# s-elkazdadi/ddp-pinocchio

Measured on AMD Instinct MI355X. Metric: DDP iterations/sec (fwd+bwd sweep), Talos nq=38 T=200, higher is better.
Workload: dtype f64

## Files before the change

ddp_pinocchio_amd/csrc/fwd.hip:

```cpp
#include <math.h>
#include <stdio.h>
#include <stdlib.h>

#include <type_traits>
#include <vector>

#include "com_cost.h"
#include "control_grav_cost.h"
#include "frame_aim_cost.h"
#include "frame_cost.h"
#include "frame_vel_cost.h"
#include "internal.h"
#include "momentum_cost.h"
#include "obstacle_cost.h"
#include "rbd.h"
#include "relative_frame_cost.h"
#include "self_collision_cost.h"
#include "state_limits.h"

namespace {

struct FwdParams {
  Dims d;
  const DevModel* model;
// ... 281 lines not shown
      const double* wu = p.wu + ((int64_t)b * T + t) * nv;
      for (int j = h; j < nv; j += NH) { const double du = u[j] - ur[j]; if (wu[j] != 0.0) su += wu[j] * du * du; }
    }
  }
  double v = 0.5 * s + 0.5 * su;
#pragma unroll
  for (int k = NH / 2; k >= 1; k /= 2) v += __shfl_xor(v, k, NH);
  return v;
}

template <bool FF, class M>
__device__ __forceinline__ double frame_lanes_sum(const FwdParams& p, const M& cm, int b, int64_t t, const double* x, int h, bool live) {
  constexpr int NH = 16;
  double s = 0;
  if (live && h < p.fc.nf) s = frame_term(p.fc, cm, FF, h, (int64_t)b * (p.d.T + 1) + t, x);
  double v = 0.5 * s;
#pragma unroll
  for (int k = NH / 2; k >= 1; k /= 2) v += __shfl_xor(v, k, NH);
  return v;
}

template <bool FF, class M>
__device__ __forceinline__ double frame_orient_lanes_sum(const FwdParams& p, const M& cm, int b, int64_t t, const double* x, int h, bool live) {
  constexpr int NH = 16;
  static_assert(2 * DDP_HIP_MAX_COST_FRAMES <= NH, "a lane per frame and kind of term");
  double s = 0;
  if (live) {
    if (h < DDP_HIP_MAX_COST_FRAMES) { if (h < p.fc.nf && p.fc.target) s = frame_term(p.fc, cm, FF, h, (int64_t)b * (p.d.T + 1) + t, x); }
    else if (h - DDP_HIP_MAX_COST_FRAMES < p.fc.nf) s = frame_orient_term(p.fc, cm, FF, h - DDP_HIP_MAX_COST_FRAMES, (int64_t)b * (p.d.T + 1) + t, x);
  }
  double v = 0.5 * s;
#pragma unroll
  for (int k = NH / 2; k >= 1; k /= 2) v += __shfl_xor(v, k, NH);
  return v;
}

template <bool FF>
__device__ __forceinline__ double limit_lanes_sum(const FwdParams& p, int b, int64_t t, const double* x, int h, bool live) {
  const int nv = (int)p.d.nv, n = 2 * nv, nq = (int)p.d.nx - nv, r0 = FF ? 6 : 0;
  constexpr int NH = 16;
  const int64_t bt1 = (int64_t)b * (p.d.T + 1) + t;
  const double* w = p.sl.weight + bt1 * n;
  const double* lo = p.sl.lo + bt1 * n;
  const double* hi = p.sl.hi + bt1 * n;
  double s = 0;
  if (live)
    for (int i = r0 + h; i < n; i += NH) {
      const double wi = w[i];
      if (wi == 0.0) continue;
      const double e = limit_excess(x[limit_coord(i, nv, nq)], lo[i], hi[i]);
      if (e != 0.0) s += wi * e * e;
    }
  double v = 0.5 * s;
#pragma unroll
  for (int k = NH / 2; k >= 1; k /= 2) v += __shfl_xor(v, k, NH);
  return v;
}

template <int NJ>
struct FwdLat2Lds {
  static constexpr int NC = 4, NH = 16, n = 2 * NJ + 1, nu = NJ;
  double state[rbd::ABA_LDS_SLOTS * (NJ + NJ / 8) * NC];
  double K[nu * n];
  double k[nu], uo[nu], xo[n];
  double dx[NC * n], x[NC * n], u[NC * nu], qdd[NC * nu];
  rbd::CoopModel<NJ> model;
};

template <int NJ>
struct FwdLat2LdsBox : FwdLat2Lds<NJ> {
  double lo[NJ], hi[NJ];
};

template <int NJ>
struct FwdPipeLds {
  static constexpr int NC = 2, NH = 16, n = 2 * NJ + 1, nu = NJ;
  double rec[2][rbd::ABA_PIPE_QSLOTS * NJ * NC];
  double z[rbd::ABA_PIPE_ZSLOTS * NJ * NC];
  double state[rbd::ABA_PIPE_XSLOTS * NJ * NC];
  double K[nu * n];
  double k[nu], uo[nu], xo[n];
  double dx[NC * n], x[2 * NC * n], u[NC * nu], qdd[NC * nu];
  rbd::CoopModel<NJ> model;
};
template <int NJ>
struct FwdPipeLdsBox : FwdPipeLds<NJ> {
  double lo[NJ], hi[NJ];
};

static bool fwd_use_pipe(const ddp_hip_ctx* ctx, int64_t batch, int n_alpha) {
  return !ctx->sw.fwd_no_pipe && batch * ((n_alpha + 1) / 2) <= ctx->cu_count;
}

#ifdef FWD_STAMPS
__device__ unsigned long long g_fwd_stamps[24];
#endif

template <int NJ, bool OPEN = false, bool FF = false, int COST = 0, bool BOX = false, bool PIPE = false>
__global__ __launch_bounds__(128) void forward_kernel_lat2(FwdParams p) {
  static_assert(!(OPEN && BOX), "the open-loop rollout applies U as given");
  constexpr bool TRACK = (COST & 1) != 0, FRAME = (COST & 2) != 0, LIMIT = (COST & 4) != 0, ORIENT = (COST & 8) != 0;
  static_assert(!ORIENT || FRAME, "the orientation terms are of the cost frames: bit 3 implies bit 1");
  using L = typename std::conditional<PIPE, typename std::conditional<BOX, FwdPipeLdsBox<NJ>, FwdPipeLds<NJ>>::type,
                                      typename std::conditional<BOX, FwdLat2LdsBox<NJ>, FwdLat2Lds<NJ>>::type>::type;
  constexpr int NC = L::NC, NH = L::NH;
  constexpr int n = 2 * NJ, nq = FF ? NJ + 1 : NJ, nx = nq + NJ, nu = NJ, XS = L::n;
  constexpr int K2 = nu * n / 2, KR = (K2 + 63) / 64;
  static_assert((nu * n) % 2 == 0, "K_t is moved in 16-byte words");
  extern __shared__ __attribute__((aligned(16))) double lds[];
  L& S = *reinterpret_cast<L*>(lds);
  const int na = OPEN ? 1 : p.n_alpha;
  const int groups = PIPE ? (na + NC - 1) / NC : 2;
  const int b = OPEN ? blockIdx.x : blockIdx.x / groups, half = OPEN ? 0 : blockIdx.x % groups;
  if (!OPEN && p.state[b] != 0) return;
  if (half * NC >= na) return;
  const int wave = threadIdx.x / 64, tid = threadIdx.x % 64, al0 = tid / NH, h = tid % NH;
  const int al = al0 < NC ? al0 : NC - 1;
  const int a = half * NC + al;
  const int cand = p.round * na + a;
  const bool mine = al0 < NC && a < na;
  const bool live = mine && cand <= 33;
  if (!OPEN && mine && cand > 33 && h == 0 && wave == 0) p.fw_dcost[(int64_t)b * na + a] = INFINITY;
  const double step = ldexp(1.0, -cand);
  const int64_t T = p.d.T;
  const double* xo = p.x_old + (int64_t)b * (T + 1) * nx;
  const double* uo = p.u_old + (int64_t)b * T * nu;
  double* xw = OPEN ? const_cast<double*>(p.x_old) + (int64_t)b * (T + 1) * nx : p.fw_x + ((int64_t)b * na + (a < na ? a : 0)) * (T + 1) * nx;
  double* uw = OPEN ? nullptr : p.fw_u + ((int64_t)b * na + (a < na ? a : 0)) * T * nu;
  const double* cold = p.costs_old + (int64_t)b * (T + 1);
  const double* kg = p.fb_val + (int64_t)b * T * nu;
  const double* Kg = p.fb_jac + (int64_t)b * T * nu * n;
  double* dx = S.dx + al * XS;
  double* x = S.x + al * XS;
  double* u = S.u + al * nu;
  double* qdd = S.qdd + al * nu;
  if (wave == 0) {
    const DevModel& m = *p.model;
    rbd::CoopModel<NJ>& cm = S.model;
    for (int i = tid; i < NJ; i += 64) {
      for (int k2 = 0; k2 < 21; ++k2) cm.I6[i][k2] = m.I6[i][k2];
      for (int k2 = 0; k2 < 9; ++k2) cm.Rp[i][k2] = m.Rp[i][k2];
      for (int k2 = 0; k2 < 3; ++k2) { cm.axis[i][k2] = m.axis[i][k2]; cm.pp[i][k2] = m.pp[i][k2]; }
      cm.parent[i] = m.parent[i]; cm.jtype[i] = m.jtype[i];
      cm.lvl_joint[i] = m.lvl_joint[i]; cm.child_list[i] = m.child_list[i];
      cm.lvl_start[i] = m.lvl_start[i]; cm.child_start[i] = m.child_start[i];
    }
    if (tid == 0) {
      cm.lvl_start[NJ] = m.lvl_start[NJ]; cm.child_start[NJ] = m.child_start[NJ];
      cm.n_levels = m.n_levels; cm.nv = m.nv; cm.nj = m.nj;
      cm.gravity[0] = m.gravity[0]; cm.gravity[1] = m.gravity[1]; cm.gravity[2] = m.gravity[2];
      cm.dt = m.dt; cm.c = m.c;
    }
    for (int e = tid; e < 16 * NH; e += 64) {
      const int L = e / NH, hh = e % NH;
      unsigned long long r = 255;
      if (L < m.n_levels && m.lvl_start[L] + hh < m.lvl_start[L + 1]) {
        const int j = m.lvl_joint[m.lvl_start[L] + hh];
        int ch[rbd::ROLE_MAX_CHILDREN] = {0, 0, 0};
        const int nch = m.child_start[j + 1] - m.child_start[j];
        for (int c = 0; c < nch && c < rbd::ROLE_MAX_CHILDREN; ++c) ch[c] = m.child_list[m.child_start[j] + c];
        r = rbd::coop_role(j, m.parent[j], m.jtype[j] == DDP_HIP_JOINT_REVOLUTE, nch, ch);
      }
      cm.role[e] = r;
    }
  }
  typedef double d2 __attribute__((ext_vector_type(2)));
  d2 Kreg[KR];
  double kreg = 0.0, uoreg = 0.0, xoreg0 = 0.0, xoreg1 = 0.0, coldreg = 0.0;
  [[maybe_unused]] double loreg = 0.0, hireg = 0.0;
  auto request = [&](int64_t t) {
    const int iu = tid < nu ? tid : nu - 1;
    uoreg = uo[t * nu + iu];
    if constexpr (!OPEN) {
      const d2* Kt = reinterpret_cast<const d2*>(Kg + t * nu * n);
#pragma unroll
      for (int j = 0; j < KR; ++j) { const int e = j * 64 + tid; Kreg[j] = Kt[e < K2 ? e : K2 - 1]; }
      kreg = kg[t * nu + iu];
      if constexpr (BOX) { loreg = p.ctrl_lo[((int64_t)b * T + t) * nu + iu]; hireg = p.ctrl_hi[((int64_t)b * T + t) * nu + iu]; }
      xoreg0 = xo[t * nx + (tid < nx ? tid : nx - 1)];
      xoreg1 = xo[t * nx + (64 + tid < nx ? 64 + tid : nx - 1)];
      coldreg = cold[t];
    }
  };
  auto park = [&]() {
    if (tid < nu) S.uo[tid] = uoreg;
    if constexpr (!OPEN) {
      d2* Ks = reinterpret_cast<d2*>(S.K);
#pragma unroll
      for (int j = 0; j < KR; ++j) { const int e = j * 64 + tid; if (e < K2) Ks[e] = Kreg[j]; }
      if (tid < nu) S.k[tid] = kreg;
      if constexpr (BOX) { if (tid < nu) { S.lo[tid] = loreg; S.hi[tid] = hireg; } }
      if (tid < nx) S.xo[tid] = xoreg0;
      if (64 + tid < nx) S.xo[64 + tid] = xoreg1;
    }
  };
  static_assert(nx <= 128, "x_old is parked by two words per lane");
  double cold_t = 0.0, dsum = 0.0;
  const double mc = p.model->c, mdt = p.model->dt;
  if (wave == 0) {
    request(0);
    const double* x0 = OPEN ? xw : p.x_new + (int64_t)b * (T + 1) * nx;
    if (live)
      for (int i = h; i < nx; i += NH) { const double v = x0[i]; x[i] = v; if (!OPEN) xw[i] = v; }
    park();
    cold_t = coldreg;
  }
  rbd::wg_sync_lds();
  const bool lead = wave == 0;
  rbd::FwdStamp* fs = nullptr;
#ifdef FWD_STAMPS
  rbd::FwdStamp fsv{};
  if (lead || PIPE) fs = &fsv;
  fsv.last = wall_clock64();
#endif
  for (int64_t t = PIPE ? -1 : 0; t < T; ++t) {
    if constexpr (PIPE) x = S.x + ((int)(t & 1) * NC + al) * XS;
    if (lead && (!PIPE || t >= 0)) {
    if constexpr (OPEN) {
      if (live)
        for (int i = h; i < nu; i += NH) u[i] = S.uo[i];
    } else {
    if constexpr (FF) {
      if (live) {
        if (h == 0) lie::se3_difference(S.xo, x, dx);
        for (int i = 6 + h; i < NJ; i += NH) dx[i] = x[i + 1] - S.xo[i + 1];
        for (int i = h; i < NJ; i += NH) dx[NJ + i] = x[nq + i] - S.xo[nq + i];
      }
    } else {
    if (live)
      for (int i = h; i < n; i += NH) dx[i] = x[i] - S.xo[i];
    }
    rbd::coop_sync<true>();
    {
      constexpr int NR = (nu + NH - 1) / NH;
      double acc[NR];
#pragma unroll
      for (int r = 0; r < NR; ++r) acc[r] = 0.0;
      const double* Kr[NR];
#pragma unroll
      for (int r = 0; r < NR; ++r) { const int i = h + NH * r; Kr[r] = S.K + (i < nu ? i : nu - 1); }
#pragma unroll
      for (int l = 0; l < n; ++l) {
        const double d = dx[l];
#pragma unroll
        for (int r = 0; r < NR; ++r) acc[r] += Kr[r][l * nu] * d;
      }
#pragma unroll
      for (int r = 0; r < NR; ++r) {
        const int i = h + NH * r;
        if (i < nu && live) {
          double ui = S.uo[i] + step * S.k[i];
          ui += acc[r];
          if constexpr (BOX) { const double lo = S.lo[i], hi = S.hi[i]; ui = ui < lo ? lo : (ui > hi ? hi : ui); }
          u[i] = ui;
          uw[t * nu + i] = ui;
        }
      }
    }
    rbd::coop_sync<true>();
    FSTAMP(fs, 0);
    double c_track = 0.0;
    if constexpr (TRACK) c_track = track_lanes_sum<FF>(p, b, t, x, u, h, live);
    if constexpr (FRAME && !ORIENT) c_track += frame_lanes_sum<FF>(p, S.model, b, t, x, h, live);
    if constexpr (ORIENT) c_track += frame_orient_lanes_sum<FF>(p, S.model, b, t, x, h, live);
    if constexpr (LIMIT) c_track += limit_lanes_sum<FF>(p, b, t, x, h, live);
    if (h == 0 && live && p.cost_inline) {
      double un = 0;
      for (int i = 0; i < nu; ++i) un += u[i] * u[i];
      double c_new = 0.5 * mc * un;
      if constexpr (TRACK || FRAME || LIMIT) c_new += c_track;
      dsum += c_new - cold_t;
    }
    }
    rbd::coop_sync<true>();
    FSTAMP(fs, 1);
    if (t + 1 < T) request(t + 1);
    FSTAMP(fs, 2);
    }
    if constexpr (PIPE) {
      double* xn = S.x + ((int)((t + 1) & 1) * NC + al) * XS;
      if (lead) {
        if (t >= 0) {
          rbd::aba_pipe_x<NJ, NC, NH, rbd::CoopModel<NJ>, FF>(S.model, S.rec[t & 1], x + nq, u, qdd, S.state, al, h, live, fs);
          if (live)
            for (int i = h; i < NJ; i += NH) {
              const double vn = x[nq + i] + qdd[i] * mdt;
              xn[nq + i] = vn;
              xw[(t + 1) * nx + nq + i] = vn;
            }
          FSTAMP(fs, 7);
          if (t + 1 < T) { park(); cold_t = coldreg; }
          FSTAMP(fs, 8);
        }
      } else {
        if (t >= 0) {
          if constexpr (FF) {
            if (live && h == 0) {
              double dq[6], q7[7];
#pragma unroll
              for (int k = 0; k < 6; ++k) dq[k] = mdt * x[nq + k];
              lie::se3_integrate(x, dq, q7);
#pragma unroll
              for (int k = 0; k < 7; ++k) xn[k] = q7[k];
            }
            if (live)
              for (int i = 6 + h; i < NJ; i += NH) { const double vo = mdt * x[nq + i]; xn[i + 1] = x[i + 1] + vo; }
          } else {
            if (live)
              for (int i = h; i < NJ; i += NH) { const double vo = mdt * x[NJ + i]; xn[i] = x[i] + vo; }
          }
          rbd::coop_sync<true>();
          FSTAMP(fs, 0);
        }
        if (t + 1 < T) rbd::aba_pipe_q<NJ, NC, NH, rbd::CoopModel<NJ>, FF>(S.model, xn, S.rec[(t + 1) & 1], S.z, al, h, live, fs);
      }
      rbd::wg_sync_lds();
      FSTAMP(fs, lead ? 3 : 5);
      if (lead && t >= 0 && live)
        for (int i = h; i < nq; i += NH) xw[(t + 1) * nx + i] = xn[i];
      continue;
    }
    rbd::aba_tree_coop2w<NJ, NC, NH, rbd::CoopModel<NJ>, FF>(S.model, x, x + nq, u, qdd, S.state, al, h, live, wave, fs);
    if (!lead) continue;
    if constexpr (FF) {
      double q7[7];
      if (live && h == 0) {
        double dq[6];
#pragma unroll
        for (int k = 0; k < 6; ++k) dq[k] = mdt * x[nq + k];
        lie::se3_integrate(x, dq, q7);
      }
      rbd::coop_sync<true>();
      if (live) {
        for (int i = 6 + h; i < NJ; i += NH) { const double vo = mdt * x[nq + i]; const double qn = x[i + 1] + vo; x[i + 1] = qn; xw[(t + 1) * nx + i + 1] = qn; }
        for (int i = h; i < NJ; i += NH) { const double vn = x[nq + i] + qdd[i] * mdt; x[nq + i] = vn; xw[(t + 1) * nx + nq + i] = vn; }
        if (h == 0) {
#pragma unroll
          for (int k = 0; k < 7; ++k) { x[k] = q7[k]; xw[(t + 1) * nx + k] = q7[k]; }
        }
      }
    } else {
    if (live)
      for (int i = h; i < NJ; i += NH) {
        const double vo = mdt * x[NJ + i];
        const double qn = x[i] + vo;
        const double vn = x[NJ + i] + qdd[i] * mdt;
        x[i] = qn; x[NJ + i] = vn;
        xw[(t + 1) * nx + i] = qn; xw[(t + 1) * nx + NJ + i] = vn;
      }
    }
    FSTAMP(fs, 7);
    if (t + 1 < T) { park(); cold_t = coldreg; }
    rbd::coop_sync<true>();
    FSTAMP(fs, 8);
  }
#ifdef FWD_STAMPS
  if (tid == 0 && blockIdx.x == 0)
    for (int i = 0; i < 12; ++i) g_fwd_stamps[12 * wave + i] = PIPE || lead ? fsv.acc[i] : 0;
#endif
  if constexpr (PIPE) x = S.x + ((int)(T & 1) * NC + al) * XS;
  double c_term = 0.0;
  if constexpr (TRACK) { if (lead) c_term = track_lanes_sum<FF>(p, b, T, x, u, h, live); }
  if constexpr (FRAME && !ORIENT) { if (lead) c_term += frame_lanes_sum<FF>(p, S.model, b, T, x, h, live); }
  if constexpr (ORIENT) { if (lead) c_term += frame_orient_lanes_sum<FF>(p, S.model, b, T, x, h, live); }
  if constexpr (LIMIT) { if (lead) c_term += limit_lanes_sum<FF>(p, b, T, x, h, live); }
  if (!OPEN && h == 0 && live && lead && p.cost_inline) {
    dsum += c_term - cold[T];
    p.fw_dcost[(int64_t)b * na + a] = dsum;
  }
}

template <int NJ, int FRAME = 0, bool LIMIT = false>
__global__ void cand_cost_kernel(FwdParams p) {
  const int64_t gid = (int64_t)blockIdx.x * blockDim.x + threadIdx.x;
  const int64_t T = p.d.T;
  const int na = p.n_alpha;
  if (gid >= p.d.batch * na * (T + 1)) return;
  const int64_t t = gid % (T + 1);
  const int a = (int)((gid / (T + 1)) % na);
  const int b = (int)(gid / ((T + 1) * na));
  if (p.state[b] != 0 || p.round * na + a > 33) return;
  const DevModel& m = *p.model;
  const int nx = m.nq + m.nv, nu = m.nv;
  const double* xs = p.fw_x + (((int64_t)b * na + a) * (T + 1) + t) * nx;
  double x[2 * NJ + 1], u[NJ];
  for (int i = 0; i < nx; ++i) x[i] = xs[i];
  double* out = p.fw_cost + ((int64_t)b * na + a) * (T + 1) + t;
  if (t == T) { *out = terminal_cost<FRAME, LIMIT>(p, m, b, x); return; }
  const double* us = p.fw_u + (((int64_t)b * na + a) * T + t) * nu;
  for (int i = 0; i < nu; ++i) u[i] = us[i];
  *out = stage_cost<NJ, FRAME, LIMIT>(p, m, b, t, x, u, p.mu[b]);
}
__global__ void cand_sum_kernel(FwdParams p) {
  const int gid = blockIdx.x * blockDim.x + threadIdx.x;
  const int na = p.n_alpha;
  if (gid >= p.d.batch * na) return;
  const int b = gid / na, a = gid % na;
  if (p.state[b] != 0 || p.round * na + a > 33) return;
  const int64_t T = p.d.T;
  const double* cold = p.costs_old + (int64_t)b * (T + 1);
  const double* cnew = p.fw_cost + ((int64_t)b * na + a) * (T + 1);
  double dsum = 0.0;
  for (int64_t t = 0; t < T; ++t) dsum += cnew[t] - cold[t];
  dsum += cnew[T] - cold[T];
  p.fw_dcost[(int64_t)b * na + a] = dsum;
}

struct CostPair {
  int64_t traj, b, bt1;
  int t;
  bool skip, live;
};
__device__ __forceinline__ CostPair cost_pair_decode(int64_t e, int64_t count, int32_t T1, int32_t na, const int32_t* state, int32_t round) {
  CostPair p{0, 0, 0, 0, true, e < count};
  if (p.live) {
    p.traj = e / T1;
    p.t = (int)(e % T1);
    p.b = p.traj / na;
    if (state && (state[p.b] != 0 || round * na + (int)(p.traj % na) > 33)) p.live = false;
    p.bt1 = p.b * T1 + p.t;
  }
  p.skip = !p.live;
  return p;
}
__device__ __forceinline__ void cost_pair_store(double* out, int64_t e, double sum, bool any, int32_t add) {
  if (add) { if (any) out[e] += sum; }
  else out[e] = sum;
}
template <int L, bool MIN, class Form>
__device__ __forceinline__ void pair_lanes_fold(double* s_term, int32_t* s_formed, int n, const double* xs, int64_t traj_stride, int64_t count,
                                                int32_t T1, int32_t nx, int32_t na, const int32_t* state, int32_t round, double* out, int32_t add,
                                                Form form) {
  const int tid = threadIdx.x, g = tid / L, k = tid % L;
  const int64_t e = (int64_t)blockIdx.x * (64 / L) + g;
  const CostPair pr = cost_pair_decode(e, count, T1, na, state, round);
  double term = MIN ? INFINITY : 0.0;
  bool formed = false;
  if (pr.live && k < n) formed = form(k, pr.bt1, xs + pr.traj * traj_stride + (int64_t)pr.t * nx, &term);
  s_term[tid] = term;
  if (!MIN) s_formed[tid] = formed ? 1 : 0;
  __syncthreads();
  if (k != 0 || pr.skip) return;
  double acc = MIN ? INFINITY : 0.0;
  bool any = false;
  for (int i = 0; i < n; ++i) {
    if (MIN) acc = rbd::obstacle_min(acc, s_term[tid + i]);
    else if (s_formed[tid + i]) { acc += s_term[tid + i]; any = true; }
  }
  cost_pair_store(out, e, acc, any, add);
// ... 345 lines not shown
#define LAT2_ROW(FF, COST) {{&forward_kernel_lat2<38, false, FF, COST, false, false>, &forward_kernel_lat2<38, false, FF, COST, false, true>}, \
                            {&forward_kernel_lat2<38, false, FF, COST, true, false>, &forward_kernel_lat2<38, false, FF, COST, true, true>}}
  static const Lat2Fn table[2][12][2][2] = {{LAT2_ROW(false, 0), LAT2_ROW(false, 1), LAT2_ROW(false, 2), LAT2_ROW(false, 3),
                                             LAT2_ROW(false, 4), LAT2_ROW(false, 5), LAT2_ROW(false, 6), LAT2_ROW(false, 7),
                                             LAT2_ROW(false, 10), LAT2_ROW(false, 11), LAT2_ROW(false, 14), LAT2_ROW(false, 15)},
                                            {LAT2_ROW(true, 0), LAT2_ROW(true, 1), LAT2_ROW(true, 2), LAT2_ROW(true, 3),
                                             LAT2_ROW(true, 4), LAT2_ROW(true, 5), LAT2_ROW(true, 6), LAT2_ROW(true, 7),
                                             LAT2_ROW(true, 10), LAT2_ROW(true, 11), LAT2_ROW(true, 14), LAT2_ROW(true, 15)}};
#undef LAT2_ROW
  if ((cost & 8) && !(cost & 2)) return nullptr;
  const int slot = (cost & 8) ? 8 + (cost & 1) + ((cost & 4) ? 2 : 0) : cost & 7;
  return table[ff ? 1 : 0][slot][box ? 1 : 0][pipe ? 1 : 0];
}
Lat2Fn lat2_open_kernel(bool ff, bool pipe) {
  static const Lat2Fn table[2][2] = {{&forward_kernel_lat2<38, true, false, 0, false, false>, &forward_kernel_lat2<38, true, false, 0, false, true>},
                                     {&forward_kernel_lat2<38, true, true, 0, false, false>, &forward_kernel_lat2<38, true, true, 0, false, true>}};
  return table[ff ? 1 : 0][pipe ? 1 : 0];
}
size_t lat2_lds(bool box, bool pipe) {
  if (pipe) return box ? sizeof(FwdPipeLdsBox<38>) : sizeof(FwdPipeLds<38>);
  return box ? sizeof(FwdLat2LdsBox<38>) : sizeof(FwdLat2Lds<38>);
}

#define DISPATCH_NJ(nv, CALL)                 \
  do {                                        \
    if ((nv) <= 1) { CALL(1); }               \
    else if ((nv) <= 6) { CALL(6); }          \
    else if ((nv) <= 38) { CALL(38); }        \
    else { CALL(64); }                        \
  } while (0)

}

bool fwd_lat_supported(const ddp_hip_ctx* ctx) {
  const DevModel& m = ctx->model_h;
  if (m.kind != DDP_HIP_MODEL_TREE || ctx->d.nv != 38) return false;
  if (m.max_level_width > 8 || m.n_levels > 16) return false;
  for (int j = 0; j < m.nj; ++j)
    if (m.child_start[j + 1] - m.child_start[j] > rbd::ROLE_MAX_CHILDREN) return false;
  return true;
}

int fwd_setup(ddp_hip_ctx* ctx) {
  const Dims& d = ctx->d;
  const int64_t B = d.batch, na = ctx->n_alpha_max;
  HIP_TRY(hipMalloc(&ctx->fw_x, sizeof(double) * (size_t)(B * na * (d.T + 1) * d.nx)));
  HIP_TRY(hipMalloc(&ctx->fw_u, sizeof(double) * (size_t)(B * na * d.T * d.m)));
  HIP_TRY(hipMalloc(&ctx->fw_dcost, sizeof(double) * (size_t)(B * na)));
  if (d.Etot > 0) HIP_TRY(hipMalloc(&ctx->fw_cost, sizeof(double) * (size_t)(B * na * (d.T + 1))));
  HIP_TRY(hipMalloc(&ctx->step_d, sizeof(double) * (size_t)B));
  HIP_TRY(hipMalloc(&ctx->fw_dcost_acc_d, sizeof(double) * (size_t)B));
  HIP_TRY(hipMalloc(&ctx->fw_state_d, sizeof(int32_t) * (size_t)B));
  if (d.nv == 38) {
    for (int ff = 0; ff < 2; ++ff)
      for (int pipe = 0; pipe < 2; ++pipe)
        HIP_TRY(hipFuncSetAttribute(reinterpret_cast<const void*>(lat2_open_kernel(ff != 0, pipe != 0)), hipFuncAttributeMaxDynamicSharedMemorySize,
                                    (int)lat2_lds(false, pipe != 0)));
    const bool frame = (ctx->flags & DDP_HIP_FLAG_FRAME_COST) != 0, bounds = (ctx->flags & DDP_HIP_FLAG_CONTROL_BOUNDS) != 0;
    const int costs = 1 | (frame ? 2 : 0) | ((ctx->flags & DDP_HIP_FLAG_STATE_LIMITS) ? 4 : 0) |
                      ((ctx->flags & DDP_HIP_FLAG_FRAME_ORIENT_COST) ? 8 : 0);
    for (int ff = 0; ff < 2; ++ff)
      for (int cost = 0; cost < 16; ++cost)
        for (int box = 0; box < (bounds ? 2 : 1); ++box)
          for (int pipe = 0; pipe < 2; ++pipe)
            if (!(cost & ~costs) && (!(cost & 8) || (cost & 2)))
              HIP_TRY(hipFuncSetAttribute(reinterpret_cast<const void*>(lat2_kernel(ff != 0, cost, box != 0, pipe != 0)),
                                          hipFuncAttributeMaxDynamicSharedMemorySize, (int)lat2_lds(box != 0, pipe != 0)));
  }
  return DDP_HIP_OK;
}

void fwd_teardown(ddp_hip_ctx* ctx) {
  if (ctx->fw_x) (void)hipFree(ctx->fw_x);
  if (ctx->fw_u) (void)hipFree(ctx->fw_u);
  if (ctx->fw_dcost) (void)hipFree(ctx->fw_dcost);
  if (ctx->fw_cost) (void)hipFree(ctx->fw_cost);
  if (ctx->step_d) (void)hipFree(ctx->step_d);
  if (ctx->fw_dcost_acc_d) (void)hipFree(ctx->fw_dcost_acc_d);
  if (ctx->pick_pair_d) (void)hipFree(ctx->pick_pair_d);
  if (ctx->fw_state_d) (void)hipFree(ctx->fw_state_d);
}

#ifdef FWD_STAMPS
extern "C" int ddp_hip_debug_fwd_stamps(unsigned long long* out24) {
  return hipMemcpyFromSymbol(out24, HIP_SYMBOL(g_fwd_stamps), sizeof(unsigned long long) * 24) == hipSuccess ? 0 : -2;
}
#endif

extern "C" int ddp_hip_rollout(ddp_hip_ctx* ctx) {
  if (!ctx) return DDP_HIP_E_ARG;
  HIP_TRY(hipSetDevice(ctx->device));
  FwdParams p = make_params(ctx);
  if (fwd_lat_supported(ctx)) {
    const bool pipe = fwd_use_pipe(ctx, ctx->d.batch, 1);
    hipLaunchKernelGGL(lat2_open_kernel(ctx->model_h.ff != 0, pipe), dim3((unsigned)ctx->d.batch), dim3(128), lat2_lds(false, pipe), ctx->stream, p);
  } else {
    const int bs = 64;
    const unsigned grid = (unsigned)((ctx->d.batch + bs - 1) / bs);
#define CALL(NJ) hipLaunchKernelGGL((rollout_kernel<NJ>), dim3(grid), dim3(bs), 0, ctx->stream, p)
    DISPATCH_NJ(ctx->d.nv, CALL);
#undef CALL
  }
  HIP_TRY(hipGetLastError());
  HIP_TRY(hipStreamSynchronize(ctx->stream));
  return DDP_HIP_OK;
}

#define DISPATCH_COST(p, LAUNCH)                               \
  do {                                                         \
    const bool fr_ = (p).fc.target != nullptr, or_ = (p).fc.oquat != nullptr, li_ = (p).sl.weight != nullptr; \
    if (or_ && li_) LAUNCH(2, true);                           \
    else if (or_) LAUNCH(2, false);                            \
    else if (fr_ && li_) LAUNCH(1, true);                      \
    else if (li_) LAUNCH(0, true);                             \
    else if (fr_) LAUNCH(1, false);                            \
    else LAUNCH(0, false);                                     \
  } while (0)

typedef void (*AddOnLaunch)(ddp_hip_ctx* ctx, const double* xs, const double* us, int na, int64_t count, const int32_t* state, int round, double* out, int add);

template <class Kernel, class Dev, class... Mid>
static void launch_add_on(Kernel kernel, const Dev& dev, int lanes, ddp_hip_ctx* ctx, const double* xs, int na, int64_t count, const int32_t* state,
                          int round, double* out, int add, Mid... mid) {
  const Dims& d = ctx->d;
  const int64_t per = 64 / lanes;
  hipLaunchKernelGGL(kernel, dim3((unsigned)((count + per - 1) / per)), dim3(64), 0, ctx->stream, dev, ctx->model_d, xs, (d.T + 1) * d.nx, count,
                     (int32_t)(d.T + 1), (int32_t)d.nx, (int32_t)na, mid..., state, (int32_t)round, out, (int32_t)add);
}

static void launch_com_cost(ddp_hip_ctx* ctx, const double* xs, const double* us, int na, int64_t count, const int32_t* state, int round, double* out, int add) {
  int32_t lpe = 8;
  while (lpe < ctx->model_h.nj) lpe *= 2;
  launch_add_on(com_cost_kernel, com_cost_dev(ctx), lpe, ctx, xs, na, count, state, round, out, add, lpe);
}
static void launch_frame_vel_cost(ddp_hip_ctx* ctx, const double* xs, const double* us, int na, int64_t count, const int32_t* state, int round, double* out, int add) {
  launch_add_on(frame_vel_cost_kernel, frame_vel_cost_dev(ctx), DDP_HIP_MAX_COST_FRAMES, ctx, xs, na, count, state, round, out, add);
}
static void launch_momentum_cost(ddp_hip_ctx* ctx, const double* xs, const double* us, int na, int64_t count, const int32_t* state, int round, double* out, int add) {
  int32_t lpe = 8;
  while (lpe < ctx->model_h.nj) lpe *= 2;
  launch_add_on(momentum_cost_kernel, momentum_cost_dev(ctx), lpe, ctx, xs, na, count, state, round, out, add, lpe);
}
static void launch_relative_frame_cost(ddp_hip_ctx* ctx, const double* xs, const double* us, int na, int64_t count, const int32_t* state, int round, double* out, int add) {
  launch_add_on(relative_frame_cost_kernel, relative_frame_dev(ctx), DDP_HIP_MAX_FRAME_PAIRS, ctx, xs, na, count, state, round, out, add);
}
static void launch_control_grav_cost(ddp_hip_ctx* ctx, const double* xs, const double* us, int na, int64_t count, const int32_t* state, int round, double* out, int add) {
  int32_t lpe = 8;
  while (lpe < ctx->model_h.nj) lpe *= 2;
  launch_add_on(control_grav_cost_kernel, control_grav_dev(ctx), lpe, ctx, xs, na, count, state, round, out, add, lpe, us, ctx->d.T * ctx->d.m);
}
static void launch_frame_aim_cost(ddp_hip_ctx* ctx, const double* xs, const double* us, int na, int64_t count, const int32_t* state, int round, double* out, int add) {
  launch_add_on(frame_aim_cost_kernel, frame_aim_dev(ctx), DDP_HIP_MAX_AIM_FRAMES, ctx, xs, na, count, state, round, out, add);
}
static void launch_obstacle_cost(ddp_hip_ctx* ctx, const double* xs, const double* us, int na, int64_t count, const int32_t* state, int round, double* out, int add) {
  launch_add_on(obstacle_cost_kernel, obstacle_cost_dev(ctx), DDP_HIP_MAX_COLLISION_POINTS, ctx, xs, na, count, state, round, out, add);
}
static void launch_self_collision_cost(ddp_hip_ctx* ctx, const double* xs, const double* us, int na, int64_t count, const int32_t* state, int round, double* out, int add) {
  launch_add_on(self_collision_cost_kernel, self_collision_dev(ctx), DDP_HIP_MAX_COLLISION_POINTS, ctx, xs, na, count, state, round, out, add);
}

struct AddOnTerm {
  int term;
  AddOnLaunch launch;
};
static const AddOnTerm kAddOn[] = {{COST_COM, launch_com_cost},
                                   {COST_FRAME_VEL, launch_frame_vel_cost},
                                   {COST_MOMENTUM, launch_momentum_cost},
                                   {COST_RELATIVE_FRAME, launch_relative_frame_cost},
                                   {COST_CONTROL_GRAV, launch_control_grav_cost},
                                   {COST_FRAME_AIM, launch_frame_aim_cost},
                                   {COST_OBSTACLE, launch_obstacle_cost},
                                   {COST_SELF_COLLISION, launch_self_collision_cost}};

static int launch_cost(ddp_hip_ctx* ctx, FwdParams& p, int which) {
  const int bs = 64;
  const int64_t total = ctx->d.batch * (ctx->d.T + 1);
  const unsigned grid = (unsigned)((total + bs - 1) / bs);
#define CALL(NJ) hipLaunchKernelGGL((cost_kernel<NJ, FR, LI>), dim3(grid), dim3(bs), 0, ctx->stream, p, which)
// ... 30 lines not shown
  hipLaunchKernelGGL(obstacle_clearance_kernel, dim3((unsigned)((total + per - 1) / per)), dim3(64), 0, ctx->stream, ob, ctx->model_d,
                     which == 0 ? p.x_old : p.x_new, total, (int32_t)ctx->d.nx, ctx->ob_clear_d);
  HIP_TRY(hipGetLastError());
  HIP_TRY(hipMemcpyAsync(out, ctx->ob_clear_d, sizeof(double) * (size_t)total, hipMemcpyDeviceToHost, ctx->stream));
  HIP_TRY(hipStreamSynchronize(ctx->stream));
  return DDP_HIP_OK;
}

extern "C" int ddp_hip_self_collision_clearance(ddp_hip_ctx* ctx, int which, double* out) {
  if (!ctx) return DDP_HIP_E_ARG;
  if (!(ctx->flags & DDP_HIP_FLAG_SELF_COLLISION_COST)) return DDP_HIP_E_UNSUPPORTED;
  if (!out || (which != 0 && which != 1) || ctx->sc_npair == 0) return DDP_HIP_E_ARG;
  HIP_TRY(hipSetDevice(ctx->device));
  const FwdParams p = make_params(ctx);
  const SelfCollisionDev sc = self_collision_dev(ctx, true);
  const int64_t total = ctx->d.batch * (ctx->d.T + 1);
  const int64_t per = 64 / DDP_HIP_MAX_COLLISION_POINTS;
  hipLaunchKernelGGL(self_collision_clearance_kernel, dim3((unsigned)((total + per - 1) / per)), dim3(64), 0, ctx->stream, sc, ctx->model_d,
                     which == 0 ? p.x_old : p.x_new, total, (int32_t)ctx->d.nx, ctx->sc_clear_d);
  HIP_TRY(hipGetLastError());
  HIP_TRY(hipMemcpyAsync(out, ctx->sc_clear_d, sizeof(double) * (size_t)total, hipMemcpyDeviceToHost, ctx->stream));
  HIP_TRY(hipStreamSynchronize(ctx->stream));
  return DDP_HIP_OK;
}

extern "C" int ddp_hip_relative_frame_error(ddp_hip_ctx* ctx, int which, double* out) {
  if (!ctx) return DDP_HIP_E_ARG;
  if (!(ctx->flags & DDP_HIP_FLAG_RELATIVE_FRAME_COST)) return DDP_HIP_E_UNSUPPORTED;
  if (!out || (which != 0 && which != 1) || ctx->rf_np == 0) return DDP_HIP_E_ARG;
  HIP_TRY(hipSetDevice(ctx->device));
  const FwdParams p = make_params(ctx);
  const RelativeFrameDev rf = relative_frame_dev(ctx, true);
  const int64_t total = ctx->d.batch * (ctx->d.T + 1);
  hipLaunchKernelGGL(relative_frame_error_kernel, dim3((unsigned)((total * rf.np + 63) / 64)), dim3(64), 0, ctx->stream, rf, ctx->model_d,
                     which == 0 ? p.x_old : p.x_new, total, (int32_t)ctx->d.nx, ctx->rf_err_d);
  HIP_TRY(hipGetLastError());
  HIP_TRY(hipMemcpyAsync(out, ctx->rf_err_d, sizeof(double) * (size_t)(total * rf.np * 6), hipMemcpyDeviceToHost, ctx->stream));
  HIP_TRY(hipStreamSynchronize(ctx->stream));
  return DDP_HIP_OK;
}

extern "C" int ddp_hip_frame_aim_error(ddp_hip_ctx* ctx, int which, double* out) {
  if (!ctx) return DDP_HIP_E_ARG;
  if (!(ctx->flags & DDP_HIP_FLAG_FRAME_AIM_COST)) return DDP_HIP_E_UNSUPPORTED;
  if (!out || (which != 0 && which != 1) || ctx->fa_nf == 0) return DDP_HIP_E_ARG;
  HIP_TRY(hipSetDevice(ctx->device));
  const FwdParams p = make_params(ctx);
  const FrameAimDev fa = frame_aim_dev(ctx, true);
  const int64_t total = ctx->d.batch * (ctx->d.T + 1);
  hipLaunchKernelGGL(frame_aim_error_kernel, dim3((unsigned)((total * fa.nf + 63) / 64)), dim3(64), 0, ctx->stream, fa, ctx->model_d,
                     which == 0 ? p.x_old : p.x_new, total, (int32_t)ctx->d.nx, ctx->fa_err_d);
  HIP_TRY(hipGetLastError());
  HIP_TRY(hipMemcpyAsync(out, ctx->fa_err_d, sizeof(double) * (size_t)(total * fa.nf * 2), hipMemcpyDeviceToHost, ctx->stream));
  HIP_TRY(hipStreamSynchronize(ctx->stream));
  return DDP_HIP_OK;
}

extern "C" int ddp_hip_forward(ddp_hip_ctx* ctx, const double* mu, int32_t n_alpha, double* step_out, double* dcost_out) {
  if (!ctx || !mu || !step_out || n_alpha < 0 || n_alpha > ctx->n_alpha_max) return DDP_HIP_E_ARG;
  const bool no_linesearch = n_alpha == 0;
  if (no_linesearch) n_alpha = 1;
  const Dims& d = ctx->d;
  const int64_t B = d.batch;
  HIP_TRY(hipSetDevice(ctx->device));
  if (ctx->flags & DDP_HIP_FLAG_CONTROL_BOUNDS) { const int rc_ = box_check(ctx); if (rc_ != DDP_HIP_OK) return rc_; }
  HIP_TRY(hipMemcpyAsync(ctx->mu_d, mu, sizeof(double) * (size_t)B, hipMemcpyHostToDevice, ctx->stream));
  std::vector<int32_t> state((size_t)B);
  for (int64_t b = 0; b < B; ++b) state[(size_t)b] = ctx->active_h[(size_t)b] ? 0 : 1;
  HIP_TRY(hipMemcpyAsync(ctx->fw_state_d, state.data(), sizeof(int32_t) * (size_t)B, hipMemcpyHostToDevice, ctx->stream));
  FwdParams p = make_params(ctx);
  p.n_alpha = n_alpha;
  p.no_linesearch = no_linesearch ? 1 : 0;
  int rc = launch_cost(ctx, p, 0);
  if (rc != DDP_HIP_OK) return rc;
  const int bs = 64;
  const unsigned grid = (unsigned)((B * n_alpha + bs - 1) / bs);
  bool floor_hit = false;
  for (int round = 0; round * n_alpha <= 33; ++round) {
    p.round = round;
    prof_begin(ctx, DDP_HIP_K_FWD_ROLLOUT);
    const bool lat_path = fwd_lat_supported(ctx) && n_alpha <= 8;
    if (lat_path) {
      const bool pipe = fwd_use_pipe(ctx, B, n_alpha);
      const dim3 g((unsigned)(pipe ? B * ((n_alpha + 1) / 2) : 2 * B)), blk(128);
      const int cost = p.cost_inline ? (p.track ? 1 : 0) | (p.fc.target ? 2 : 0) | (p.sl.weight ? 4 : 0) | (p.fc.oquat ? 10 : 0) : 0;
      const bool box = p.ctrl_lo != nullptr;
      hipLaunchKernelGGL(lat2_kernel(ctx->model_h.ff != 0, cost, box, pipe), g, blk, lat2_lds(box, pipe), ctx->stream, p);
      if (!p.cost_inline) {
        const dim3 gc((unsigned)((B * n_alpha * (d.T + 1) + 63) / 64));
#define LAUNCH(F, L) hipLaunchKernelGGL((cand_cost_kernel<38, F, L>), gc, dim3(64), 0, ctx->stream, p)
        DISPATCH_COST(p, LAUNCH);
#undef LAUNCH
        hipLaunchKernelGGL(cand_sum_kernel, dim3((unsigned)((B * n_alpha + 63) / 64)), dim3(64), 0, ctx->stream, p);
      }
    } else {
#define CALL(NJ) hipLaunchKernelGGL((forward_kernel<NJ, FR, LI>), dim3(grid), dim3(bs), 0, ctx->stream, p)
#define LAUNCH(F, L) do { constexpr int FR = F; constexpr bool LI = L; DISPATCH_NJ(d.nv, CALL); } while (0)
      DISPATCH_COST(p, LAUNCH);
#undef LAUNCH
#undef CALL
    }
    prof_end(ctx, DDP_HIP_K_FWD_ROLLOUT);
    for (const AddOnTerm& a : kAddOn) {
      const CostBlock& k = ctx->cost[a.term];
      if (!k.live) continue;
      a.launch(ctx, p.fw_x, p.fw_u, n_alpha, B * n_alpha * (d.T + 1), p.state, round, k.cand, 0);
      hipLaunchKernelGGL(com_sum_kernel, dim3((unsigned)((B * n_alpha + 63) / 64)), dim3(64), 0, ctx->stream, k.cand, p.fw_dcost, p.state,
                         (int32_t)B, (int32_t)n_alpha, (int32_t)round, d.T);
    }
    hipLaunchKernelGGL(select_kernel, dim3((unsigned)B), dim3(256), 0, ctx->stream, p);
    HIP_TRY(hipGetLastError());
    HIP_TRY(hipMemcpyAsync(state.data(), ctx->fw_state_d, sizeof(int32_t) * (size_t)B, hipMemcpyDeviceToHost, ctx->stream));
    HIP_TRY(hipStreamSynchronize(ctx->stream));
    bool searching = false;
    for (int64_t b = 0; b < B; ++b) { searching |= state[(size_t)b] == 0; floor_hit |= state[(size_t)b] == 2; }
    if (!searching) break;
  }
  HIP_TRY(hipMemcpyAsync(step_out, ctx->step_d, sizeof(double) * (size_t)B, hipMemcpyDeviceToHost, ctx->stream));
  if (dcost_out)
    HIP_TRY(hipMemcpyAsync(dcost_out, ctx->fw_dcost_acc_d, sizeof(double) * (size_t)B, hipMemcpyDeviceToHost, ctx->stream));
  HIP_TRY(hipStreamSynchronize(ctx->stream));
  return floor_hit ? DDP_HIP_EV_LINESEARCH_FLOOR : DDP_HIP_OK;
}
```

ddp_pinocchio_amd/csrc/rbd.h:

```cpp
#pragma once

#include "internal.h"
#include "lie.h"

namespace rbd {

__device__ __forceinline__ void cross3(const double* a, const double* b, double* c) {
  c[0] = a[1] * b[2] - a[2] * b[1];
  c[1] = a[2] * b[0] - a[0] * b[2];
  c[2] = a[0] * b[1] - a[1] * b[0];
}
__device__ __forceinline__ double dot3(const double* a, const double* b) { return a[0] * b[0] + a[1] * b[1] + a[2] * b[2]; }
__device__ __forceinline__ void sym3_mv(const double* S, const double* x, double* y) {
  y[0] = S[0] * x[0] + S[1] * x[1] + S[3] * x[2];
  y[1] = S[1] * x[0] + S[2] * x[1] + S[4] * x[2];
  y[2] = S[3] * x[0] + S[4] * x[1] + S[5] * x[2];
}
__device__ __forceinline__ void mv3(const double* A, const double* x, double* y) {
  y[0] = A[0] * x[0] + A[1] * x[1] + A[2] * x[2];
  y[1] = A[3] * x[0] + A[4] * x[1] + A[5] * x[2];
  y[2] = A[6] * x[0] + A[7] * x[1] + A[8] * x[2];
}
__device__ __forceinline__ void mtv3(const double* A, const double* x, double* y) {
  y[0] = A[0] * x[0] + A[3] * x[1] + A[6] * x[2];
// ... 1004 lines not shown
#pragma unroll
        for (int k = 0; k < 6; ++k) accp[k] = S(par, oV + k);
      }
      step_accel_in(E, R, par >= 0, accp, m.gravity, ap);
      if (FF && i == 0) {
        double IAr[21], pAr[6];
#pragma unroll
        for (int k = 0; k < 21; ++k) IAr[k] = S(i, oZ + k);
#pragma unroll
        for (int k = 0; k < 6; ++k) pAr[k] = S(i, oP + k);
        step_accel_ff_root(IAr, pAr, tau, cb, ap, qdd);
      } else {
        qdd[VI(i)] = step_accel(U, cb, S(i, oT), S(i, oD), m.axis[i], role_rev(rr), ap);
      }
#pragma unroll
      for (int k = 0; k < 6; ++k) S(i, oV + k) = ap[k];
    }
    coop_sync<true>();
  }
  FSTAMP(fs, 6);
}

constexpr int ABA_PIPE_QSLOTS = 41;
constexpr int ABA_PIPE_ZSLOTS = 21;
constexpr int ABA_PIPE_XSLOTS = 19;

template <int NJ, int TPB, int NH, class M, bool FF = false>
__device__ __forceinline__ void aba_pipe_q(const M& m, const double* q, double* rec, double* zst, int cand, int h, bool live,
                                           FwdStamp* fs = nullptr) {
  const int nj = FF ? m.nv - 5 : m.nv;
  auto Q = [&](int joint, int slot) -> double& { return rec[(joint * ABA_PIPE_QSLOTS + slot) * TPB + cand]; };
  auto Z = [&](int joint, int slot) -> double& { return zst[(joint * ABA_PIPE_ZSLOTS + slot) * TPB + cand]; };
  constexpr int oE = 0, oR = 9, oU = 12, oD = 18, oA = 19;
  const int NL = m.n_levels;
  if (live)
    for (int i = h; i < nj; i += NH) {
      double E[9], R[3];
      step_place<FF>(m, i, q, E, R);
#pragma unroll
      for (int k = 0; k < 9; ++k) Q(i, oE + k) = E[k];
#pragma unroll
      for (int k = 0; k < 3; ++k) Q(i, oR + k) = R[k];
    }
  coop_sync<true>();
  FSTAMP(fs, 3);
  for (int L = NL - 1; L >= 0; --L) {
    const unsigned long long rr = m.role[L * NH + h];
    if (live && role_joint(rr) != 255) {
      const int i = role_joint(rr);
      double IA[21], U[6];
#pragma unroll
      for (int k = 0; k < 21; ++k) IA[k] = m.I6[i][k];
      step_add_children<21>(rr, IA, [&](int c, int k) { return Z(c, k); });
      FSTAMP(fs, 9);
      if (FF && i == 0) {
#pragma unroll
        for (int k = 0; k < 21; ++k) Q(i, oA + k) = IA[k];
      } else {
        const double dinv = step_U(IA, m.axis[i], role_rev(rr), U);
        FSTAMP(fs, 10);
#pragma unroll
        for (int k = 0; k < 6; ++k) Q(i, oU + k) = U[k];
        Q(i, oD) = dinv;
        if (role_parent(rr) >= 0) {
          double E[9], R[3], Ia[21], Zc[21];
#pragma unroll
          for (int k = 0; k < 9; ++k) E[k] = Q(i, oE + k);
#pragma unroll
          for (int k = 0; k < 3; ++k) R[k] = Q(i, oR + k);
          step_Ia(IA, U, dinv, Ia);
#pragma unroll
          for (int k = 0; k < 21; ++k) Q(i, oA + k) = Ia[k];
          step_inertia_up(E, R, Ia, Zc);
#pragma unroll
          for (int k = 0; k < 21; ++k) Z(i, k) = Zc[k];
        }
      }
    }
    FSTAMP(fs, 11);
    coop_sync<true>();
  }
}

template <int NJ, int TPB, int NH, class M, bool FF = false>
__device__ __forceinline__ void aba_pipe_x(const M& m, const double* rec, const double* v, const double* tau, double* qdd,
                                           double* xst, int cand, int h, bool live, FwdStamp* fs = nullptr) {
  auto VI = [](int i) { return FF ? i + 5 : i; };
  auto Q = [&](int joint, int slot) -> const double& { return rec[(joint * ABA_PIPE_QSLOTS + slot) * TPB + cand]; };
  auto S = [&](int joint, int slot) -> double& { return xst[(joint * ABA_PIPE_XSLOTS + slot) * TPB + cand]; };
  constexpr int oE = 0, oR = 9, oU = 12, oD = 18, oA = 19;
  constexpr int oC = 0, oP = 6, oT = 12, oV = 13;
  const int NL = m.n_levels;
  for (int L = 0; L < NL; ++L) {
    const unsigned long long rr = m.role[L * NH + h];
    if (live && role_joint(rr) != 255) {
      const int i = role_joint(rr);
      double E[9], R[3], vel[6], vp[6], cb[6], pA[6];
#pragma unroll
      for (int k = 0; k < 9; ++k) E[k] = Q(i, oE + k);
#pragma unroll
      for (int k = 0; k < 3; ++k) R[k] = Q(i, oR + k);
      const int par = role_parent(rr);
      if (par >= 0) {
#pragma unroll
        for (int k = 0; k < 6; ++k) vp[k] = S(par, oV + k);
      }
      step_velocity(E, R, m.axis[i], role_rev(rr), FF && i == 0, v + (FF && i == 0 ? 0 : VI(i)), par >= 0, vp, m.I6[i], vel, cb, pA);
#pragma unroll
      for (int k = 0; k < 6; ++k) { S(i, oV + k) = vel[k]; S(i, oC + k) = cb[k]; S(i, oP + k) = pA[k]; }
    }
    coop_sync<true>();
  }
  FSTAMP(fs, 4);
  for (int L = NL - 1; L >= 0; --L) {
    const unsigned long long rr = m.role[L * NH + h];
    if (live && role_joint(rr) != 255) {
      const int i = role_joint(rr);
      double pAi[6];
#pragma unroll
      for (int k = 0; k < 6; ++k) pAi[k] = S(i, oP + k);
      step_add_children<6>(rr, pAi, [&](int c, int k) { return S(c, oP + k); });
      if (FF && i == 0) {
#pragma unroll
        for (int k = 0; k < 6; ++k) S(i, oP + k) = pAi[k];
      } else {
        const double ui = step_u(pAi, m.axis[i], role_rev(rr), tau[VI(i)]);
        S(i, oT) = ui;
        if (role_parent(rr) >= 0) {
          double E[9], R[3], U[6], cb[6], Ia[21], fp[6];
#pragma unroll
          for (int k = 0; k < 9; ++k) E[k] = Q(i, oE + k);
#pragma unroll
          for (int k = 0; k < 3; ++k) R[k] = Q(i, oR + k);
#pragma unroll
          for (int k = 0; k < 6; ++k) { U[k] = Q(i, oU + k); cb[k] = S(i, oC + k); }
#pragma unroll
          for (int k = 0; k < 21; ++k) Ia[k] = Q(i, oA + k);
          step_force_up(E, R, pAi, cb, U, Q(i, oD), ui, Ia, fp);
#pragma unroll
          for (int k = 0; k < 6; ++k) S(i, oP + k) = fp[k];
        }
      }
    }
    coop_sync<true>();
  }
  FSTAMP(fs, 5);
  for (int L = 0; L < NL; ++L) {
    const unsigned long long rr = m.role[L * NH + h];
    if (live && role_joint(rr) != 255) {
      const int i = role_joint(rr);
      double E[9], R[3], ap[6], accp[6], U[6], cb[6];
#pragma unroll
      for (int k = 0; k < 9; ++k) E[k] = Q(i, oE + k);
#pragma unroll
      for (int k = 0; k < 3; ++k) R[k] = Q(i, oR + k);
#pragma unroll
      for (int k = 0; k < 6; ++k) { U[k] = Q(i, oU + k); cb[k] = S(i, oC + k); }
      const int par = role_parent(rr);
      if (par >= 0) {
#pragma unroll
        for (int k = 0; k < 6; ++k) accp[k] = S(par, oV + k);
      }
      step_accel_in(E, R, par >= 0, accp, m.gravity, ap);
      if (FF && i == 0) {
        double IAr[21], pAr[6];
#pragma unroll
        for (int k = 0; k < 21; ++k) IAr[k] = Q(i, oA + k);
#pragma unroll
        for (int k = 0; k < 6; ++k) pAr[k] = S(i, oP + k);
        step_accel_ff_root(IAr, pAr, tau, cb, ap, qdd);
      } else {
        qdd[VI(i)] = step_accel(U, cb, S(i, oT), Q(i, oD), m.axis[i], role_rev(rr), ap);
      }
#pragma unroll
      for (int k = 0; k < 6; ++k) S(i, oV + k) = ap[k];
    }
    coop_sync<true>();
  }
  FSTAMP(fs, 6);
}

}
```

Before: 797.8.

## Add a third control wave to overlap control law with ABA velocity pass

In the pipelined forward rollout, a third wavefront now computes the feedback control u_t, the per-step costs and the parking of the next step's gains. The lead wave runs the ABA velocity sweep in parallel and waits on an LDS flag only when the backward pass needs tau. This takes the control-law and cost work off the lead wave's critical path, at the price of a larger block (192 threads), spin-waiting on LDS, and possible lower occupancy. Some cost configurations are excluded from the new mode.

Result: faster. 807.6 (median of 6 runs) (+1.2%).

```diff
diff --git a/ddp_pinocchio_amd/csrc/fwd.hip b/ddp_pinocchio_amd/csrc/fwd.hip
--- a/ddp_pinocchio_amd/csrc/fwd.hip
+++ b/ddp_pinocchio_amd/csrc/fwd.hip
@@ -387,6 +387,7 @@
   double k[nu], uo[nu], xo[n];
   double dx[NC * n], x[2 * NC * n], u[NC * nu], qdd[NC * nu];
   rbd::CoopModel<NJ> model;
+  int u_step;
 };
 template <int NJ>
 struct FwdPipeLdsBox : FwdPipeLds<NJ> {
@@ -397,12 +398,17 @@
   return !ctx->sw.fwd_no_pipe && batch * ((n_alpha + 1) / 2) <= ctx->cu_count;
 }
 
+constexpr bool fwd_pipe_assist(bool open, bool ff, int cost, bool box) {
+  if (open || box) return true;
+  return ff ? cost != 3 && cost != 6 && cost != 7 : cost != 3 && cost != 10;
+}
+
 #ifdef FWD_STAMPS
-__device__ unsigned long long g_fwd_stamps[24];
+__device__ unsigned long long g_fwd_stamps[36];
 #endif
 
 template <int NJ, bool OPEN = false, bool FF = false, int COST = 0, bool BOX = false, bool PIPE = false>
-__global__ __launch_bounds__(128) void forward_kernel_lat2(FwdParams p) {
+__global__ __launch_bounds__(PIPE && fwd_pipe_assist(OPEN, FF, COST, BOX) ? 192 : 128) void forward_kernel_lat2(FwdParams p) {
   static_assert(!(OPEN && BOX), "the open-loop rollout applies U as given");
   constexpr bool TRACK = (COST & 1) != 0, FRAME = (COST & 2) != 0, LIMIT = (COST & 4) != 0, ORIENT = (COST & 8) != 0;
   static_assert(!ORIENT || FRAME, "the orientation terms are of the cost frames: bit 3 implies bit 1");
@@ -419,13 +425,15 @@
   const int b = OPEN ? blockIdx.x : blockIdx.x / groups, half = OPEN ? 0 : blockIdx.x % groups;
   if (!OPEN && p.state[b] != 0) return;
   if (half * NC >= na) return;
+  constexpr bool ASSIST = PIPE && fwd_pipe_assist(OPEN, FF, COST, BOX);
+  constexpr int CTRL = ASSIST ? 2 : 0;
   const int wave = threadIdx.x / 64, tid = threadIdx.x % 64, al0 = tid / NH, h = tid % NH;
   const int al = al0 < NC ? al0 : NC - 1;
   const int a = half * NC + al;
   const int cand = p.round * na + a;
   const bool mine = al0 < NC && a < na;
   const bool live = mine && cand <= 33;
-  if (!OPEN && mine && cand > 33 && h == 0 && wave == 0) p.fw_dcost[(int64_t)b * na + a] = INFINITY;
+  if (!OPEN && mine && cand > 33 && h == 0 && wave == CTRL) p.fw_dcost[(int64_t)b * na + a] = INFINITY;
   const double step = ldexp(1.0, -cand);
   const int64_t T = p.d.T;
   const double* xo = p.x_old + (int64_t)b * (T + 1) * nx;
@@ -500,18 +508,20 @@
     }
   };
   static_assert(nx <= 128, "x_old is parked by two words per lane");
+  auto post_u = [&](int64_t t) { if constexpr (ASSIST) { if (tid == 0) rbd::lds_post(&S.u_step, (int)t); } };
   double cold_t = 0.0, dsum = 0.0;
   const double mc = p.model->c, mdt = p.model->dt;
-  if (wave == 0) {
+  if (wave == CTRL) {
     request(0);
     const double* x0 = OPEN ? xw : p.x_new + (int64_t)b * (T + 1) * nx;
     if (live)
       for (int i = h; i < nx; i += NH) { const double v = x0[i]; x[i] = v; if (!OPEN) xw[i] = v; }
     park();
     cold_t = coldreg;
+    if constexpr (ASSIST) { if (tid == 0) S.u_step = -1; }
   }
   rbd::wg_sync_lds();
-  const bool lead = wave == 0;
+  const bool lead = wave == 0, ctrl = wave == CTRL;
   rbd::FwdStamp* fs = nullptr;
 #ifdef FWD_STAMPS
   rbd::FwdStamp fsv{};
@@ -520,10 +530,11 @@
 #endif
   for (int64_t t = PIPE ? -1 : 0; t < T; ++t) {
     if constexpr (PIPE) x = S.x + ((int)(t & 1) * NC + al) * XS;
-    if (lead && (!PIPE || t >= 0)) {
+    if (ctrl && (!PIPE || t >= 0)) {
     if constexpr (OPEN) {
       if (live)
         for (int i = h; i < nu; i += NH) u[i] = S.uo[i];
+      if constexpr (ASSIST) { rbd::coop_sync<true>(); post_u(t); }
     } else {
     if constexpr (FF) {
       if (live) {
@@ -563,6 +574,7 @@
       }
     }
     rbd::coop_sync<true>();
+    post_u(t);
     FSTAMP(fs, 0);
     double c_track = 0.0;
     if constexpr (TRACK) c_track = track_lanes_sum<FF>(p, b, t, x, u, h, live);
@@ -586,7 +598,8 @@
       double* xn = S.x + ((int)((t + 1) & 1) * NC + al) * XS;
       if (lead) {
         if (t >= 0) {
-          rbd::aba_pipe_x<NJ, NC, NH, rbd::CoopModel<NJ>, FF>(S.model, S.rec[t & 1], x + nq, u, qdd, S.state, al, h, live, fs);
+          rbd::aba_pipe_x<NJ, NC, NH, rbd::CoopModel<NJ>, FF>(S.model, S.rec[t & 1], x + nq, u, qdd, S.state, al, h, live, fs,
+                                                              [&]() { if constexpr (ASSIST) rbd::lds_await(&S.u_step, (int)t); });
           if (live)
             for (int i = h; i < NJ; i += NH) {
               const double vn = x[nq + i] + qdd[i] * mdt;
@@ -594,9 +607,14 @@
               xw[(t + 1) * nx + nq + i] = vn;
             }
           FSTAMP(fs, 7);
-          if (t + 1 < T) { park(); cold_t = coldreg; }
-          FSTAMP(fs, 8);
+          if constexpr (!ASSIST) {
+            if (t + 1 < T) { park(); cold_t = coldreg; }
+            FSTAMP(fs, 8);
+          }
         }
+      } else if (ASSIST && ctrl) {
+        if (t >= 0 && t + 1 < T) { park(); cold_t = coldreg; }
+        FSTAMP(fs, 8);
       } else {
         if (t >= 0) {
           if constexpr (FF) {
@@ -620,7 +638,7 @@
         if (t + 1 < T) rbd::aba_pipe_q<NJ, NC, NH, rbd::CoopModel<NJ>, FF>(S.model, xn, S.rec[(t + 1) & 1], S.z, al, h, live, fs);
       }
       rbd::wg_sync_lds();
-      FSTAMP(fs, lead ? 3 : 5);
+      FSTAMP(fs, wave == 1 ? 5 : 3);
       if (lead && t >= 0 && live)
         for (int i = h; i < nq; i += NH) xw[(t + 1) * nx + i] = xn[i];
       continue;
@@ -665,11 +683,11 @@
 #endif
   if constexpr (PIPE) x = S.x + ((int)(T & 1) * NC + al) * XS;
   double c_term = 0.0;
-  if constexpr (TRACK) { if (lead) c_term = track_lanes_sum<FF>(p, b, T, x, u, h, live); }
-  if constexpr (FRAME && !ORIENT) { if (lead) c_term += frame_lanes_sum<FF>(p, S.model, b, T, x, h, live); }
-  if constexpr (ORIENT) { if (lead) c_term += frame_orient_lanes_sum<FF>(p, S.model, b, T, x, h, live); }
-  if constexpr (LIMIT) { if (lead) c_term += limit_lanes_sum<FF>(p, b, T, x, h, live); }
-  if (!OPEN && h == 0 && live && lead && p.cost_inline) {
+  if constexpr (TRACK) { if (ctrl) c_term = track_lanes_sum<FF>(p, b, T, x, u, h, live); }
+  if constexpr (FRAME && !ORIENT) { if (ctrl) c_term += frame_lanes_sum<FF>(p, S.model, b, T, x, h, live); }
+  if constexpr (ORIENT) { if (ctrl) c_term += frame_orient_lanes_sum<FF>(p, S.model, b, T, x, h, live); }
+  if constexpr (LIMIT) { if (ctrl) c_term += limit_lanes_sum<FF>(p, b, T, x, h, live); }
+  if (!OPEN && h == 0 && live && ctrl && p.cost_inline) {
     dsum += c_term - cold[T];
     p.fw_dcost[(int64_t)b * na + a] = dsum;
   }
@@ -1181,8 +1199,8 @@
 }
 
 #ifdef FWD_STAMPS
-extern "C" int ddp_hip_debug_fwd_stamps(unsigned long long* out24) {
-  return hipMemcpyFromSymbol(out24, HIP_SYMBOL(g_fwd_stamps), sizeof(unsigned long long) * 24) == hipSuccess ? 0 : -2;
+extern "C" int ddp_hip_debug_fwd_stamps(unsigned long long* out36) {
+  return hipMemcpyFromSymbol(out36, HIP_SYMBOL(g_fwd_stamps), sizeof(unsigned long long) * 36) == hipSuccess ? 0 : -2;
 }
 #endif
 
@@ -1192,7 +1210,7 @@
   FwdParams p = make_params(ctx);
   if (fwd_lat_supported(ctx)) {
     const bool pipe = fwd_use_pipe(ctx, ctx->d.batch, 1);
-    hipLaunchKernelGGL(lat2_open_kernel(ctx->model_h.ff != 0, pipe), dim3((unsigned)ctx->d.batch), dim3(128), lat2_lds(false, pipe), ctx->stream, p);
+    hipLaunchKernelGGL(lat2_open_kernel(ctx->model_h.ff != 0, pipe), dim3((unsigned)ctx->d.batch), dim3(pipe && fwd_pipe_assist(true, ctx->model_h.ff != 0, 0, false) ? 192 : 128), lat2_lds(false, pipe), ctx->stream, p);
   } else {
     const int bs = 64;
     const unsigned grid = (unsigned)((ctx->d.batch + bs - 1) / bs);
@@ -1389,9 +1407,10 @@
     const bool lat_path = fwd_lat_supported(ctx) && n_alpha <= 8;
     if (lat_path) {
       const bool pipe = fwd_use_pipe(ctx, B, n_alpha);
-      const dim3 g((unsigned)(pipe ? B * ((n_alpha + 1) / 2) : 2 * B)), blk(128);
+      const dim3 g((unsigned)(pipe ? B * ((n_alpha + 1) / 2) : 2 * B));
       const int cost = p.cost_inline ? (p.track ? 1 : 0) | (p.fc.target ? 2 : 0) | (p.sl.weight ? 4 : 0) | (p.fc.oquat ? 10 : 0) : 0;
       const bool box = p.ctrl_lo != nullptr;
+      const dim3 blk(pipe && fwd_pipe_assist(false, ctx->model_h.ff != 0, cost, box) ? 192 : 128);
       hipLaunchKernelGGL(lat2_kernel(ctx->model_h.ff != 0, cost, box, pipe), g, blk, lat2_lds(box, pipe), ctx->stream, p);
       if (!p.cost_inline) {
         const dim3 gc((unsigned)((B * n_alpha * (d.T + 1) + 63) / 64));
diff --git a/ddp_pinocchio_amd/csrc/rbd.h b/ddp_pinocchio_amd/csrc/rbd.h
--- a/ddp_pinocchio_amd/csrc/rbd.h
+++ b/ddp_pinocchio_amd/csrc/rbd.h
@@ -1110,9 +1110,19 @@
   }
 }
 
-template <int NJ, int TPB, int NH, class M, bool FF = false>
+__device__ __forceinline__ void lds_post(int* word, int value) {
+  asm volatile("s_waitcnt lgkmcnt(0)" ::: "memory");
+  *(volatile int*)word = value;
+}
+__device__ __forceinline__ void lds_await(const int* word, int value) {
+  while (__builtin_amdgcn_readfirstlane(*(volatile const int*)word) != value) __builtin_amdgcn_s_sleep(1);
+  asm volatile("" ::: "memory");
+}
+struct NoHandOff { __device__ __forceinline__ void operator()() const {} };
+
+template <int NJ, int TPB, int NH, class M, bool FF = false, class HandOff = NoHandOff>
 __device__ __forceinline__ void aba_pipe_x(const M& m, const double* rec, const double* v, const double* tau, double* qdd,
-                                           double* xst, int cand, int h, bool live, FwdStamp* fs = nullptr) {
+                                           double* xst, int cand, int h, bool live, FwdStamp* fs = nullptr, HandOff tau_ready = HandOff()) {
   auto VI = [](int i) { return FF ? i + 5 : i; };
   auto Q = [&](int joint, int slot) -> const double& { return rec[(joint * ABA_PIPE_QSLOTS + slot) * TPB + cand]; };
   auto S = [&](int joint, int slot) -> double& { return xst[(joint * ABA_PIPE_XSLOTS + slot) * TPB + cand]; };
@@ -1140,6 +1150,8 @@
     coop_sync<true>();
   }
   FSTAMP(fs, 4);
+  tau_ready();
+  FSTAMP(fs, 0);
   for (int L = NL - 1; L >= 0; --L) {
     const unsigned long long rr = m.role[L * NH + h];
     if (live && role_joint(rr) != 255) {
```
